# miha-stopar/Plonky3-mobile

Hardware: AMD Instinct MI355X
Metric: fib_air proofs/sec (higher is better)
Workload: dtype u32 (BabyBear Montgomery, 31-bit modular)

## Files before the change

### plonky3-mobile_amd/csrc/c_api.hip

```cpp
#include "../../include/p3hip.h"

#include <atomic>
#include <chrono>
#include <condition_variable>
#include <mutex>
#include <deque>
#include <thread>
#include <cctype>
#include <cstdio>
#include <cstring>

#include "bb31.hip.h"
#include "challenger.h"
#include "common.h"
#include "mmcs.h"
#include "prover.h"
#include "pcs_verifier_dev.h"
#include "verifier_dev.h"
#include "rng.h"

namespace p3 {
bool take_error(std::string* out);
}
using namespace p3;
// ... 257 lines not shown
        int rc = get_context(&cx);
        if (rc) return rc;
        return fib_trace((hipStream_t)stream, a, b, n, d_out);
    });
}

int p3hip_poseidon2_permute_dev(uint32_t* d_states, size_t n, void* stream) {
    return guarded([&]() -> int {
        if (n && !d_states) return fail(ERR_BAD_ARG, "null state pointer");
        if (misaligned(d_states, 4)) return fail(ERR_BAD_ARG, "poseidon2_permute: d_states must be 4-byte aligned");
        Context* cx;
        int rc = get_context(&cx);
        if (rc) return rc;
        if (misaligned(d_states, 16)) return poseidon2_permute_states_variant((hipStream_t)stream, d_states, n, 3);
        return poseidon2_permute_states((hipStream_t)stream, d_states, n);
    });
}
int p3hip_poseidon2_permute(uint32_t* states, size_t n) {
    return guarded([&]() -> int {
        if (!n) return OK;
        if (!states) return fail(ERR_BAD_ARG, "null state pointer");
        Context* cx;
        int rc = get_context(&cx);
        if (rc) return rc;
        hipStream_t stream = nullptr;
        rc = cx->ws(stream, 2).reserve(n * 64);
        if (rc) return rc;
        P3_HIP(hipMemcpy(cx->ws(stream, 2).ptr, states, n * 64, hipMemcpyHostToDevice));
        rc = poseidon2_permute_states(stream, cx->ws(stream, 2).as<uint32_t>(), n);
        if (rc) return rc;
        P3_HIP(hipMemcpy(states, cx->ws(stream, 2).ptr, n * 64, hipMemcpyDeviceToHost));
        return OK;
    });
}

int p3hip_poseidon2_permute_variant_dev(uint32_t* d_states, size_t n, int variant, void* stream) {
    return guarded([&]() -> int {
        if (n && !d_states) return fail(ERR_BAD_ARG, "null state pointer");
        if (variant < 0 || variant > 3)
            return fail(ERR_BAD_ARG, "poseidon2 variant: 0 = int32, 1 = fp64, 2 = fp64 one state per quad, 3 = int32 one state per 16 lanes");
        if (n > ((size_t)1 << 26)) return fail(ERR_BAD_ARG, "poseidon2 variant: at most 2^26 states per call");
        if (!n) return OK;
        if (misaligned(d_states, variant == 3 ? 4 : 16))
            return fail(ERR_BAD_ARG, "poseidon2 variant: d_states must be 16-byte aligned (4-byte for variant 3)");
        Context* cx;
        int rc = get_context(&cx);
        if (rc) return rc;
        return poseidon2_permute_states_variant((hipStream_t)stream, d_states, n, variant);
    });
}
int p3hip_poseidon2_f64_probe_dev(const double* d_in, uint32_t* d_out, size_t n, int mode, void* stream) {
    return guarded([&]() -> int {
        if (n && (!d_in || !d_out)) return fail(ERR_BAD_ARG, "null pointer");
        if (mode < 0 || mode > 3)
            return fail(ERR_BAD_ARG, "probe mode: 0 = permutation, 1 = internal rounds, 2 = reduce, 3 = permutation, one state per quad");
        if (n > ((size_t)1 << 26)) return fail(ERR_BAD_ARG, "probe: at most 2^26 states per call");
        if (!n) return OK;
        if (misaligned(d_in, 8)) return fail(ERR_BAD_ARG, "probe: d_in holds doubles and must be 8-byte aligned");
        Context* cx;
        int rc = get_context(&cx);
        if (rc) return rc;
        return poseidon2_f64_probe((hipStream_t)stream, d_in, d_out, n, mode);
    });
}
int p3hip_field_probe_dev(int op, const void* d_in, void* d_out, size_t n, void* stream) {
    return guarded([&]() -> int { return field_probe((hipStream_t)stream, op, d_in, d_out, n); });
}
int p3hip_field_probe_host(int op, const void* in, void* out, size_t n) {
    return guarded([&]() -> int { return field_probe_host(op, in, out, n); });
}

}
struct p3hip_tree {
    Tree* t;
};
extern "C" {

static int commit_async_kind(int kind, const uint32_t* const* d_mats, const size_t* heights, const size_t* widths,
                             size_t n_mats, p3hip_tree_t** tree_out, void* stream) {
    return guarded([&]() -> int {
        if (!tree_out) return fail(ERR_BAD_ARG, "mmcs_commit: null tree_out");
        Context* cx;
        int rc = get_context(&cx);
        if (rc) return rc;
        Tree* t = nullptr;
        rc = mmcs_commit((hipStream_t)stream, d_mats, heights, widths, n_mats, &t, nullptr, nullptr, kind, nullptr, cx->profile);
        if (rc) return rc;
        *tree_out = new p3hip_tree{t};
        return OK;
    });
}
int p3hip_mmcs_commit_async_dev(const uint32_t* const* d_mats, const size_t* heights, const size_t* widths,
                                size_t n_mats, p3hip_tree_t** tree_out, void* stream) {
    return commit_async_kind(HASH_POSEIDON2, d_mats, heights, widths, n_mats, tree_out, stream);
}
int p3hip_mmcs_commit_hash_dev(int hash, const uint32_t* const* d_mats, const size_t* heights, const size_t* widths,
                               size_t n_mats, uint32_t root_out[8], p3hip_tree_t** tree_out, void* stream) {
    if (!root_out) return fail(ERR_BAD_ARG, "mmcs_commit: null root_out");
    int rc = commit_async_kind(hash, d_mats, heights, widths, n_mats, tree_out, stream);
    if (rc) return rc;
    rc = p3hip_mmcs_root(*tree_out, root_out, stream);
    if (rc) { p3hip_mmcs_free(*tree_out); *tree_out = nullptr; }
    return rc;
}
size_t p3hip_mmcs_layer_words(size_t max_height) { return mmcs_layer_words(max_height); }
int p3hip_mmcs_commit_into_dev(int hash, const uint32_t* const* d_mats, const size_t* heights, const size_t* widths, size_t n_mats,
                               uint32_t* d_layers, p3hip_tree_t** tree_out, void* stream) {
    return guarded([&]() -> int {
// ... 1124 lines not shown
```

### plonky3-mobile_amd/csrc/mmcs.hip

```cpp
#include <algorithm>

#include "common.h"
#include "mmcs.h"
#include "poseidon2.hip.h"
#include "poseidon2_coop.hip.h"
#include "poseidon2_f64.hip.h"
#include "poseidon2_q4.hip.h"
#include "keccak.hip.h"

namespace p3 {

constexpr int MAX_CLASS_MATS = 16;

struct RowSet {
    const uint32_t* ptr[MAX_CLASS_MATS];
    uint32_t width[MAX_CLASS_MATS];
    uint32_t stride[MAX_CLASS_MATS];
    uint32_t count;
    uint32_t total;
};

__device__ __forceinline__ void load_digest(const uint32_t* p, uint32_t* out8) {
    const uint4* q = reinterpret_cast<const uint4*>(p);
    uint4 a = q[0], b = q[1];
// ... 40 lines not shown
    if (r >= n_rows) return;
    uint32_t s[16];
    sponge_row(rs, r, s);
    store_digest(digests + r * 8, s);
}

__global__ void __launch_bounds__(256) compress_layer_kernel(const uint32_t* prev, uint32_t* next, uint64_t n_out,
                                                             RowSet rs, uint32_t inject) {
    if (gridDim.x <= 512u) P3_LATENCY_BOUND_KERNEL();
    uint64_t i = (uint64_t)blockIdx.x * blockDim.x + threadIdx.x;
    if (i >= n_out) return;
    uint32_t s[16];
    load_digest(prev + i * 16, s);
    load_digest(prev + i * 16 + 8, s + 8);
    p2::permute(s);
    if (inject) {
        uint32_t h[16];
        sponge_row(rs, i, h);
#pragma unroll
        for (int k = 0; k < 8; k++) s[8 + k] = h[k];
        p2::permute(s);
    }
    store_digest(next + i * 8, s);
}

__global__ void __launch_bounds__(256) tree_top_kernel(uint32_t* layer0, uint32_t n0) {
    P3_LATENCY_BOUND_KERNEL();
    extern __shared__ __attribute__((aligned(16))) uint32_t lds[];
    const uint32_t tid = threadIdx.x;
    for (uint32_t i = tid; i < n0 * 8; i += blockDim.x) lds[i] = layer0[i];
    __syncthreads();
    uint32_t* out = layer0 + (size_t)n0 * 8;
    for (uint32_t n = n0; n > 1; n >>= 1) {
        uint32_t half = n >> 1;
        uint32_t s[16];
        bool act = tid < half;
        if (act) {
#pragma unroll
            for (int k = 0; k < 16; k++) s[k] = lds[tid * 16 + k];
            p2::permute(s);
        }
        __syncthreads();
        if (act) {
#pragma unroll
            for (int k = 0; k < 8; k++) lds[tid * 8 + k] = s[k];
            store_digest(out + tid * 8, s);
        }
        __syncthreads();
        out += (size_t)half * 8;
    }
}


__global__ void __launch_bounds__(256) leaf_hash_f64_kernel(const uint32_t* mat, uint32_t width, uint64_t n_rows, uint32_t* digests) {
    if (gridDim.x <= 512u) P3_LATENCY_BOUND_KERNEL();
    uint64_t r = (uint64_t)blockIdx.x * blockDim.x + threadIdx.x;
    if (r >= n_rows) return;
    double s[16];
#pragma unroll
    for (int i = 0; i < 16; i++) s[i] = 0.0;
    const uint32_t* row = mat + r * width;
    for (uint32_t k = 0; k < width; k += 8) {
#pragma unroll
        for (int i = 0; i < 8; i++)
            if (k + i < width) s[i] = p2f::load_elem(row[k + i]);
        p2f::permute(s);
        if (k + 8 < width) {
#pragma unroll
            for (int i = 0; i < 16; i++) s[i] = p2f::reduce(s[i]);
        }
    }
    uint32_t d[8];
    const p2f::MagicRegs smk = p2f::magic_regs();
#pragma unroll
    for (int i = 0; i < 8; i++) d[i] = p2f::store_elem(s[i], smk);
    store_digest(digests + r * 8, d);
}
__global__ void __launch_bounds__(256) compress_layer_q4_kernel(const uint32_t* prev, uint32_t* next, uint64_t n_out, uint32_t prio) {
    if (prio) P3_LATENCY_BOUND_KERNEL();
    const uint32_t q = threadIdx.x & 3u;
    const uint64_t i = ((uint64_t)blockIdx.x * blockDim.x + threadIdx.x) >> 2;
    const bool act = i < n_out;
    const p2q::LaneConsts lc = p2q::lane_consts(q);
    double s[4] = {0.0, 0.0, 0.0, 0.0};
    if (act) {
        const uint4 w = *reinterpret_cast<const uint4*>(prev + i * 16 + 4 * q);
        s[0] = p2f::load_elem(w.x); s[1] = p2f::load_elem(w.y); s[2] = p2f::load_elem(w.z); s[3] = p2f::load_elem(w.w);
    }
    p2q::permute(s, lc, q == 0);
    if (act && q < 2) {
        const p2f::MagicRegs smk = p2f::magic_regs();
        *reinterpret_cast<uint4*>(next + i * 8 + 4 * q) =
            make_uint4(p2f::store_elem(s[0], smk), p2f::store_elem(s[1], smk), p2f::store_elem(s[2], smk), p2f::store_elem(s[3], smk));
    }
}
__global__ void __launch_bounds__(256) leaf_hash_q4_kernel(const uint32_t* mat, uint32_t width, uint64_t n_rows, uint32_t* digests, uint32_t prio) {
    if (prio) P3_LATENCY_BOUND_KERNEL();
    const uint32_t q = threadIdx.x & 3u;
    const uint64_t r = ((uint64_t)blockIdx.x * blockDim.x + threadIdx.x) >> 2;
    const bool act = r < n_rows;
    const p2q::LaneConsts lc = p2q::lane_consts(q);
    double s[4] = {0.0, 0.0, 0.0, 0.0};
    const uint32_t* row = mat + (act ? r : 0) * width;
    for (uint32_t k = 0; k < width; k += 8) {
        if (act && q < 2) {
#pragma unroll
            for (uint32_t i = 0; i < 4; i++)
                if (k + 4 * q + i < width) s[i] = p2f::load_elem(row[k + 4 * q + i]);
        }
        p2q::permute(s, lc, q == 0);
        if (k + 8 < width) {
#pragma unroll
            for (int i = 0; i < 4; i++) s[i] = p2f::reduce(s[i]);
        }
    }
    if (act && q < 2) {
        const p2f::MagicRegs smk = p2f::magic_regs();
        *reinterpret_cast<uint4*>(digests + r * 8 + 4 * q) =
            make_uint4(p2f::store_elem(s[0], smk), p2f::store_elem(s[1], smk), p2f::store_elem(s[2], smk), p2f::store_elem(s[3], smk));
    }
}
constexpr uint32_t LEAF_WIDE_CHUNK = 32, LEAF_WIDE_STRIDE = 36;
__global__ void __launch_bounds__(256) leaf_hash_f64_wide_kernel(const uint32_t* mat, uint32_t width, uint64_t n_rows, uint32_t* digests) {
    __shared__ __attribute__((aligned(16))) uint32_t tile[256 * LEAF_WIDE_STRIDE];
    const uint32_t tid = threadIdx.x, col = tid & 31u, rsub = tid >> 5;
    const uint64_t r0 = (uint64_t)blockIdx.x * 256u, r = r0 + tid;
    double s[16];
#pragma unroll
    for (int i = 0; i < 16; i++) s[i] = 0.0;
// ... 145 lines not shown
    p2::permute(s);
#pragma unroll
    for (int k = 0; k < 4; k++) q[k] = make_uint4(s[4 * k], s[4 * k + 1], s[4 * k + 2], s[4 * k + 3]);
}


__global__ void __launch_bounds__(256, 8) poseidon2_permute_f64_kernel(uint32_t* states, uint64_t n) {
    uint64_t i = (uint64_t)blockIdx.x * blockDim.x + threadIdx.x;
    if (i >= n) return;
    double s[16];
    uint4* q = reinterpret_cast<uint4*>(states + i * 16);
#pragma unroll
    for (int k = 0; k < 4; k++) {
        uint4 v = q[k];
        s[4 * k] = p2f::load_elem(v.x); s[4 * k + 1] = p2f::load_elem(v.y); s[4 * k + 2] = p2f::load_elem(v.z); s[4 * k + 3] = p2f::load_elem(v.w);
    }
    p2f::permute(s);
#pragma unroll
    for (int k = 0; k < 4; k++)
        q[k] = make_uint4(p2f::store_elem(s[4 * k]), p2f::store_elem(s[4 * k + 1]), p2f::store_elem(s[4 * k + 2]), p2f::store_elem(s[4 * k + 3]));
}

__global__ void poseidon2_f64_probe_kernel(const double* in, uint32_t* out, uint64_t n, int mode) {
    uint64_t i = (uint64_t)blockIdx.x * blockDim.x + threadIdx.x;
    if (i >= n) return;
    double s[16];
#pragma unroll
    for (int k = 0; k < 16; k++) s[k] = in[i * 16 + k];
    if (mode == 0) p2f::permute(s);
    else if (mode == 1) p2f::internal_rounds(s, p2f::magic_regs());
    else {
#pragma unroll
        for (int k = 0; k < 16; k++) s[k] = p2f::reduce(s[k]);
    }
#pragma unroll
    for (int k = 0; k < 16; k++) out[i * 16 + k] = p2f::store_elem(s[k]);
}
__global__ void __launch_bounds__(256) poseidon2_q4_probe_kernel(const double* in, uint32_t* out, uint64_t n) {
    const uint32_t q = threadIdx.x & 3u;
    const uint64_t i = ((uint64_t)blockIdx.x * blockDim.x + threadIdx.x) >> 2;
    const bool act = i < n;
    const p2q::LaneConsts lc = p2q::lane_consts(q);
    double s[4] = {0.0, 0.0, 0.0, 0.0};
    if (act) {
#pragma unroll
        for (int k = 0; k < 4; k++) s[k] = in[i * 16 + 4 * q + k];
    }
    p2q::permute(s, lc, q == 0);
    if (act) {
#pragma unroll
        for (int k = 0; k < 4; k++) out[i * 16 + 4 * q + k] = p2f::store_elem(s[k]);
    }
}
int poseidon2_f64_probe(hipStream_t stream, const double* d_in, uint32_t* d_out, uint64_t n, int mode) {
    if (!n) return OK;
    if (mode == 3) hipLaunchKernelGGL(poseidon2_q4_probe_kernel, dim3((uint32_t)((n * 4 + 255) / 256)), dim3(256), 0, stream, d_in, d_out, n);
    else hipLaunchKernelGGL(poseidon2_f64_probe_kernel, dim3((uint32_t)((n + 255) / 256)), dim3(256), 0, stream, d_in, d_out, n, mode);
    P3_HIP(hipGetLastError());
    return OK;
}
__global__ void __launch_bounds__(256) poseidon2_permute_q4_kernel(uint32_t* states, uint64_t n) {
    const uint32_t q = threadIdx.x & 3u;
    const uint64_t i = ((uint64_t)blockIdx.x * blockDim.x + threadIdx.x) >> 2;
    const bool act = i < n;
    const p2q::LaneConsts lc = p2q::lane_consts(q);
    double s[4] = {0.0, 0.0, 0.0, 0.0};
    uint4* mine = reinterpret_cast<uint4*>(states + (act ? i : 0) * 16 + 4 * q);
    if (act) {
        const uint4 w = *mine;
        s[0] = p2f::load_elem(w.x); s[1] = p2f::load_elem(w.y); s[2] = p2f::load_elem(w.z); s[3] = p2f::load_elem(w.w);
    }
    p2q::permute(s, lc, q == 0);
    if (act) {
        const p2f::MagicRegs smk = p2f::magic_regs();
        *mine = make_uint4(p2f::store_elem(s[0], smk), p2f::store_elem(s[1], smk), p2f::store_elem(s[2], smk), p2f::store_elem(s[3], smk));
    }
}
__global__ void __launch_bounds__(256) poseidon2_permute_coop_kernel(uint32_t* states, uint64_t n) {
    const uint32_t lane16 = threadIdx.x & 15;
    const p2c::LaneConst lc = p2c::lane_constants(lane16);
    const uint64_t i = ((uint64_t)blockIdx.x * blockDim.x + threadIdx.x) >> 4;
    const bool act = i < n;
    uint32_t v = act ? states[i * 16 + lane16] : 0u;
    v = p2c::permute(v, lc);
    if (act) states[i * 16 + lane16] = v;
}
int poseidon2_permute_states_variant(hipStream_t stream, uint32_t* d_states, uint64_t n, int variant) {
    if (!n) return OK;
    if (variant == 3) hipLaunchKernelGGL(poseidon2_permute_coop_kernel, dim3((uint32_t)((n * 16 + 255) / 256)), dim3(256), 0, stream, d_states, n);
    else if (variant == 2) hipLaunchKernelGGL(poseidon2_permute_q4_kernel, dim3((uint32_t)((n * 4 + 255) / 256)), dim3(256), 0, stream, d_states, n);
    else if (variant == 1) hipLaunchKernelGGL(poseidon2_permute_f64_kernel, dim3((uint32_t)((n + 255) / 256)), dim3(256), 0, stream, d_states, n);
    else hipLaunchKernelGGL(poseidon2_permute_kernel, dim3((uint32_t)((n + 255) / 256)), dim3(256), 0, stream, d_states, n);
    P3_HIP(hipGetLastError());
    return OK;
}

int poseidon2_permute_states(hipStream_t stream, uint32_t* d_states, uint64_t n) {
    return poseidon2_permute_states_variant(stream, d_states, n, 1);
}

__device__ __forceinline__ uint32_t rowset_elem(const RowSet& rs, uint64_t r, uint32_t k, uint32_t& m, uint32_t& base) {
    while (k - base >= rs.width[m]) { base += rs.width[m]; m++; }
    return rs.ptr[m][r * rs.stride[m] + (k - base)];
}
__device__ __forceinline__ void keccak_sponge_row(const RowSet& rs, uint64_t r, uint64_t (&st)[25]) {
#pragma unroll
    for (int i = 0; i < 25; i++) st[i] = 0;
    const uint32_t n = rs.total, n64 = (n + 1) / 2;
    uint32_t m = 0, base = 0;
// ... 435 lines not shown
    const uint64_t KCOOP_IN = profile == PROFILE_LATENCY ? (1ull << 12) : (1ull << 10);
    constexpr uint32_t KCOOP_CHUNK_LOG = 4;
    constexpr uint64_t KLANE_CHUNK = 1ull << 7;
    if (kind == HASH_KECCAK) {
        RowSet rs0 = make_rowset(*t, maxh);
        if (rs0.count == 1 && rs0.width[0] >= 68 && rs0.stride[0] == rs0.width[0])
            hipLaunchKernelGGL(keccak_leaf_wide_kernel, dim3((uint32_t)((maxh + 255) / 256)), dim3(256), 0, stream, rs0.ptr[0], rs0.width[0], maxh,
                               t->layers);
        else if (!launch_keccak_leaf_salted(stream, rs0, maxh, t->layers))
            hipLaunchKernelGGL(keccak_leaf_kernel, dim3((uint32_t)((maxh + 255) / 256)), dim3(256), 0, stream, rs0, maxh, t->layers);
        P3_HIP(hipGetLastError());
        for (size_t l = 1; l < t->layer_len.size(); l++) {
            uint64_t len = t->layer_len[l];
            RowSet rs = make_rowset(*t, len);
            if (len < COOP_MAX && !rs.count) {
                const uint64_t n_in = t->layer_len[l - 1];
                const bool coop = n_in <= KCOOP_IN;
                uint32_t levels = 0;
                while (levels < (coop ? KCOOP_CHUNK_LOG : 11u) && l + levels < t->layer_len.size() && !has_height(*t, t->layer_len[l + levels])) levels++;
                if (!coop) while (levels > 1 && (n_in >> levels) < KCOOP_IN) levels--;
                const uint32_t chunk = (uint32_t)std::min<uint64_t>(n_in, coop ? 1ull << KCOOP_CHUNK_LOG : KLANE_CHUNK);
                while ((1u << levels) > chunk) levels--;
                if (coop)
                    hipLaunchKernelGGL(keccak_tree_levels_coop_kernel, dim3((uint32_t)(n_in / chunk)), dim3(std::max<uint32_t>(64, chunk * 32)), 0,
                                       stream, t->layers + t->layer_off[l - 1], (uint32_t)n_in, chunk, levels, root_copy);
                else
                    hipLaunchKernelGGL(keccak_tree_levels_kernel, dim3((uint32_t)(n_in / chunk)), dim3(std::max<uint32_t>(64, chunk / 2)),
                                       (size_t)chunk * 32, stream, t->layers + t->layer_off[l - 1], (uint32_t)n_in, chunk, levels, root_copy);
                P3_HIP(hipGetLastError());
                if (t->layer_len[l + levels - 1] == 1) t->root_copied = root_copy != nullptr;
                l += levels - 1;
                continue;
            }
            hipLaunchKernelGGL(keccak_compress_kernel, dim3((uint32_t)((len + 255) / 256)), dim3(256), 0, stream,
                               t->layers + t->layer_off[l - 1], t->layers + t->layer_off[l], len, rs, rs.count > 0 ? 1u : 0u);
            P3_HIP(hipGetLastError());
        }
        *out = t.release();
        return OK;
    }
    {
        RowSet rs = make_rowset(*t, maxh);
        const bool dense1 = rs.count == 1 && rs.stride[0] == rs.width[0];
        if (dense1 && maxh < COOP_MAX && maxh * 16 <= 0x7fffffffull) {
            hipLaunchKernelGGL(leaf_coop_kernel, dim3((uint32_t)((maxh * 16 + 255) / 256)), dim3(256), 0, stream, rs.ptr[0],
                               rs.width[0], (uint32_t)maxh, t->layers);
        } else if (dense1 && maxh <= Q4_MAX && rs.width[0] <= 64 && (reinterpret_cast<uintptr_t>(t->layers) & 15u) == 0) {
            hipLaunchKernelGGL(leaf_hash_q4_kernel, dim3((uint32_t)((maxh * 4 + 255) / 256)), dim3(256), 0, stream, rs.ptr[0], rs.width[0], maxh,
                               t->layers, Q4_PRIO);
        } else if (dense1 && rs.width[0] >= 64) {
            hipLaunchKernelGGL(leaf_hash_f64_wide_kernel, dim3((uint32_t)((maxh + 255) / 256)), dim3(256), 0, stream, rs.ptr[0],
                               rs.width[0], maxh, t->layers);
        } else if (dense1) {
            hipLaunchKernelGGL(leaf_hash_f64_kernel, dim3((uint32_t)((maxh + 255) / 256)), dim3(256), 0, stream, rs.ptr[0],
                               rs.width[0], maxh, t->layers);
        } else if ((maxh >= COOP_MAX || (rs.count == 1 && !dense1))) {
            hipLaunchKernelGGL(leaf_hash_f64_rowset_kernel, dim3((uint32_t)((maxh + 255) / 256)), dim3(256), 0, stream, rs, maxh, t->layers);
        } else {
            hipLaunchKernelGGL(leaf_hash_kernel, dim3((uint32_t)((maxh + 255) / 256)), dim3(256), 0, stream, rs, maxh, t->layers);
        }
        P3_HIP(hipGetLastError());
    }
    for (size_t l = 1; l < t->layer_len.size();) {
        uint64_t len = t->layer_len[l];
        RowSet rs = make_rowset(*t, len);
        bool inject = rs.count > 0;
        if (!inject && len < COOP_MAX) {
            uint32_t levels = 0;
            while (levels < COOP_CHUNK_LOG && l + levels < t->layer_len.size() && !has_height(*t, t->layer_len[l + levels])) levels++;
            uint64_t n_in = t->layer_len[l - 1];
            uint32_t chunk = (uint32_t)std::min<uint64_t>(n_in, 1ull << COOP_CHUNK_LOG);
            while ((1u << levels) > chunk) levels--;
            uint32_t blocks = (uint32_t)(n_in / chunk);
            uint32_t threads = std::max<uint32_t>(64, chunk * 8);
            bool makes_root = t->layer_len[l + levels - 1] == 1;
            hipLaunchKernelGGL(tree_levels_coop_kernel, dim3(blocks), dim3(threads), 0, stream, t->layers + t->layer_off[l - 1],
                               (uint32_t)n_in, chunk, levels, makes_root ? root_copy : nullptr);
            P3_HIP(hipGetLastError());
            if (makes_root) t->root_copied = root_copy != nullptr;
            l += levels;
            continue;
        }
        if (!inject && len <= Q4_MAX) {
            hipLaunchKernelGGL(compress_layer_q4_kernel, dim3((uint32_t)((len * 4 + 255) / 256)), dim3(256), 0, stream,
                               t->layers + t->layer_off[l - 1], t->layers + t->layer_off[l], len, Q4_PRIO);
        } else if (!inject) {
            hipLaunchKernelGGL(compress_layer_f64_kernel, dim3((uint32_t)((len + 255) / 256)), dim3(256), 0, stream,
                               t->layers + t->layer_off[l - 1], t->layers + t->layer_off[l], len);
        } else {
            hipLaunchKernelGGL(compress_layer_kernel, dim3((uint32_t)((len + 255) / 256)), dim3(256), 0, stream,
                               t->layers + t->layer_off[l - 1], t->layers + t->layer_off[l], len, rs, inject ? 1u : 0u);
        }
        P3_HIP(hipGetLastError());
        l++;
    }
    *out = t.release();
    return OK;
}

int mmcs_root(hipStream_t stream, const Tree& t, uint32_t root_out[8]) {
    P3_HIP(hipMemcpyAsync(root_out, t.layers + t.layer_off.back(), 32, hipMemcpyDeviceToHost, stream));
    P3_HIP(hipStreamSynchronize(stream));
    return OK;
}

static OpenArgs make_open_args(const Tree& t) {
    OpenArgs a{};
    a.n_mats = (uint32_t)t.mats.size();
// ... 47 lines not shown
```

### plonky3-mobile_amd/csrc/poseidon2_f64.hip.h

```cpp
#pragma once
#include "poseidon2.hip.h"

namespace p2f {

constexpr double PD = 2013265921.0;
constexpr double PINV = 1.0 / 2013265921.0;

__device__ __forceinline__ double mulmod(double a, double b) {
    double h = a * b;
    double l = __fma_rn(a, b, -h);
    double q = __builtin_rint(h * PINV);
    double r = __fma_rn(-q, PD, h);
    return r + l;
}
constexpr double PM1 = 2013265920.0;
__device__ __forceinline__ double mulmod_p(double a, double b, double aP) {
    double q = __builtin_rint(b * aP);
    double t = __fma_rn(a, b, -(q * PM1));
    return t - q;
}
__device__ __forceinline__ double reduce(double x) {
    return __fma_rn(-__builtin_rint(x * PINV), PD, x);
}
__device__ __forceinline__ double add_scaled_pow2(double tot, double x, double inv) {
// ... 88 lines not shown
    auto internal_round = [&](int r) {
        s[0] = sbox7(s[0] + d_c.in[r], mk, npm1, pinv);
        const double ti = (((s[0] + s[1]) + (s[2] + s[4])) + ((s[5] + s[7]) + (s[8] + s[12]))) + s[15];
        const double tf = ((s[3] + s[6]) + (s[9] + s[10])) + ((s[11] + s[13]) + s[14]);
        const double tot = reduce(ti + fold_dyadic(tf));
        s[0] = __fma_rn(s[0], -2.0, tot);
        s[1] = tot + s[1];
        s[2] = __fma_rn(s[2], 2.0, tot);
        s[3] = __fma_rn(s[3], 0.5, tot);
        s[4] = __fma_rn(s[4], k3, tot);
        s[5] = __fma_rn(s[5], 4.0, tot);
        s[6] = __fma_rn(s[6], -0.5, tot);
        s[7] = __fma_rn(s[7], -k3, tot);
        s[8] = __fma_rn(s[8], -4.0, tot);
        s[9] = __fma_rn(s[9], i256, tot);
        s[10] = __fma_rn(s[10], i4, tot);
        s[11] = __fma_rn(s[11], i8, tot);
        s[12] = __fma_rn(s[12], -k15, tot);
        s[13] = __fma_rn(s[13], -i256, tot);
        s[14] = __fma_rn(s[14], -i16, tot);
        s[15] = __fma_rn(s[15], k15, tot);
        if (FOLD_K1 >> r & 1) { s[3] = fold_dyadic(s[3]); s[6] = fold_dyadic(s[6]); }
        if (FOLD_K8 >> r & 1) { s[9] = fold_dyadic(s[9]); s[13] = fold_dyadic(s[13]); }
        if (FOLD_K2 >> r & 1) s[10] = fold_dyadic(s[10]);
        if (FOLD_K3 >> r & 1) s[11] = fold_dyadic(s[11]);
        if (FOLD_K4 >> r & 1) s[14] = fold_dyadic(s[14]);
        if (FOLD_X2 >> r & 1) { s[1] = reduce(s[1]); s[2] = reduce(s[2]); }
        if (FOLD_X4 >> r & 1) { s[4] = reduce(s[4]); s[5] = reduce(s[5]); s[7] = reduce(s[7]); s[8] = reduce(s[8]); }
        if (FOLD_X15 >> r & 1) { s[12] = reduce(s[12]); s[15] = reduce(s[15]); }
    };
#pragma unroll
    for (int r = 0; r < 13; r++) internal_round(r);
}

__device__ __forceinline__ void permute(double (&s)[16]) {
    const MagicRegs mk = magic_regs();
    const double npm1 = d_c.neg_pm1, pinv = d_c.pinv;
    external_linear(s);
    _Pragma("clang loop unroll(disable)")
    for (int r = 0; r < 4; r++) {
#pragma unroll
        for (int i = 0; i < 16; i++) s[i] = sbox7(s[i] + d_c.ext[r][i], mk, npm1, pinv);
        external_linear(s);
    }
    internal_rounds(s, mk);
    _Pragma("clang loop unroll(disable)")
    for (int r = 4; r < 8; r++) {
#pragma unroll
        for (int i = 0; i < 16; i++) s[i] = sbox7(s[i] + d_c.ext[r][i], mk, npm1, pinv);
        external_linear(s);
    }
}

__device__ __forceinline__ double load_elem(uint32_t monty) { return (double)bb::from_monty(monty); }
constexpr double R_MOD_P = 268435454.0;
constexpr double R_MOD_P_OVER_P = 268435454.0 / 2013265921.0;
__device__ __forceinline__ uint32_t store_elem(double v, const MagicRegs& k) {
    const double r = mulmod_m(R_MOD_P, v, R_MOD_P_OVER_P, k, d_c.neg_pm1);
    const uint32_t w = (uint32_t)(int32_t)r;
    return min(w, w + bb::P);
}
__device__ __forceinline__ uint32_t store_elem(double v) { return store_elem(v, magic_regs()); }

}
```

### plonky3-mobile_amd/csrc/prover.hip

```cpp
#include <chrono>
#include <cstddef>
#include <deque>
#include <memory>
#include <cstring>

#include "bb31.hip.h"
#include "challenger.h"
#include "common.h"
#include "keccak.hip.h"
#include "mmcs.h"
#include "poseidon2.hip.h"
#include "poseidon2_f64.hip.h"
#include "prover.h"
#include "rng.h"
#include "rng_dev.hip.h"
#include "transcript.hip.h"

namespace p3 {

using bb::Ext;

__device__ __forceinline__ uint32_t tl(const TwoLevelTable& t, uint32_t e) {
    return bb::mul(t.lo[e & ((1u << t.T) - 1u)], t.hi[e >> t.T]);
}
// ... 170 lines not shown
    uint32_t* ro;
    const DevState* ds;
    uint32_t big;
};
__global__ void __launch_bounds__(256) reduced_openings_kernel(ReducedArgs a) {
    uint32_t j = blockIdx.x * blockDim.x + threadIdx.x;
    if (j >= a.big) return;
    const DevState* __restrict__ ds = a.ds;
    uint2 t = a.lde_t[j];
    uint4 q = a.lde_q[j];
    Ext u, w;
#pragma unroll
    for (int c = 0; c < 4; c++) {
        u.c[c] = bb::add(bb::add(bb::dot2(ds->alp[4].c[c], q.x, ds->alp[5].c[c], q.y), bb::dot2(ds->alp[6].c[c], q.z, ds->alp[7].c[c], q.w)),
                         bb::mul(ds->alp[1].c[c], t.y));
        w.c[c] = bb::dot2(ds->alp[2].c[c], t.x, ds->alp[3].c[c], t.y);
    }
    u.c[0] = bb::add(u.c[0], t.x);
    Ext e0 = ld_ext(a.d0 + 4 * (size_t)j), e1 = ld_ext(a.d1 + 4 * (size_t)j);
    Ext r = bb::add(bb::mul(bb::sub(ds->y02, u), e0), bb::mul(bb::sub(ds->y1, w), e1));
    st_ext(a.ro + 4 * (size_t)j, r);
}

__global__ void __launch_bounds__(256) fri_fold_kernel(TwoLevelTable inv_roots , const uint32_t* in,
                                                       uint32_t* out, uint32_t half, uint32_t log_half,
                                                       const DevState* __restrict__ ds, uint32_t round, uint32_t one_half) {
    if (gridDim.x <= 512u) P3_LATENCY_BOUND_KERNEL();
    uint32_t i = blockIdx.x * blockDim.x + threadIdx.x;
    if (i >= half) return;
    const Ext half_beta = ds->half_beta[round];
    Ext lo = ld_ext(in + 8 * (size_t)i), hi = ld_ext(in + 8 * (size_t)i + 4);
    uint32_t p = tl(inv_roots, brev(i, log_half));
    Ext s = bb::scale(bb::add(lo, hi), one_half);
    Ext d = bb::mul(bb::scale(half_beta, p), bb::sub(lo, hi));
    st_ext(out + 4 * (size_t)i, bb::add(s, d));
}

__global__ void __launch_bounds__(256) fri_fold_rollin_kernel(TwoLevelTable inv_roots , const uint32_t* in,
                                                              const uint32_t* __restrict__ ro, uint32_t* out, uint32_t half,
                                                              uint32_t log_half, const DevState* __restrict__ ds, uint32_t round,
                                                              uint32_t one_half) {
    if (gridDim.x <= 512u) P3_LATENCY_BOUND_KERNEL();
    uint32_t i = blockIdx.x * blockDim.x + threadIdx.x;
    if (i >= half) return;
    const Ext half_beta = ds->half_beta[round];
    const Ext beta2 = bb::sqr(bb::add(half_beta, half_beta));
    Ext lo = ld_ext(in + 8 * (size_t)i), hi = ld_ext(in + 8 * (size_t)i + 4), e = ld_ext(ro + 4 * (size_t)i);
    uint32_t p = tl(inv_roots, brev(i, log_half));
    Ext s = bb::scale(bb::add(lo, hi), one_half);
    Ext d = bb::mul(bb::scale(half_beta, p), bb::sub(lo, hi));
    st_ext(out + 4 * (size_t)i, bb::add(bb::add(s, d), bb::mul(beta2, e)));
}

__global__ void __launch_bounds__(256, 8) grind_kernel(DevState* ds, uint32_t mask, uint32_t base) {
    uint32_t w = base + blockIdx.x * blockDim.x + threadIdx.x;
    if (w >= bb::P) return;
    if (base + blockIdx.x * blockDim.x > *(volatile uint32_t*)&ds->grind_result) return;
    const uint32_t pos = ds->n_in;
    double s[16];
#pragma unroll
    for (int i = 0; i < 16; i++) s[i] = p2f::load_elem((i < 8 && (uint32_t)i < pos) ? ds->inb[i & 7] : ds->st[i]);
#pragma unroll
    for (int i = 0; i < 8; i++) s[i] = (i == (int)pos) ? (double)w : s[i];
    p2f::permute(s);
    if ((bb::from_monty(p2f::store_elem(s[7])) & mask) == 0) atomicMin(&ds->grind_result, w);
}

__global__ void __launch_bounds__(256) grind_keccak_kernel(DevState* ds, uint32_t mask, uint32_t base) {
    uint32_t w = base + blockIdx.x * blockDim.x + threadIdx.x;
    if (w >= bb::P) return;
    if (base + blockIdx.x * blockDim.x > *(volatile uint32_t*)&ds->grind_result) return;
    const KeccakGrindArgs& a = ds->kgrind;
    const uint32_t wm = bb::to_monty(w);
    uint64_t st[25];
#pragma unroll
    for (int i = 0; i < 25; i++) st[i] = a.state[i];
    for (uint32_t blk = 0; blk < a.n_blocks; blk++) {
#pragma unroll
        for (int i = 0; i < 17; i++) {
            uint64_t lane = a.block[blk][i];
            const int32_t rel = (int32_t)(a.wpos) - (int32_t)(blk * 136 + i * 8);
            if (rel > -4 && rel < 8) {
                const uint64_t v = (uint64_t)wm;
                lane ^= rel >= 0 ? (v << (8 * rel)) : (v >> (8 * -rel));
            }
            st[i] ^= lane;
        }
        if (blk + 1 == a.n_blocks) kk::permute_digest(st);
        else kk::permute(st);
    }
    bool ok = false;
#pragma unroll
    for (int t = 0; t < 8; t++) {
        const uint64_t lane = st[3 - t / 2];
        const uint32_t hi_or_lo = (t & 1) ? (uint32_t)lane : (uint32_t)(lane >> 32);
        const uint32_t v = __builtin_bswap32(hi_or_lo) & 0x7fffffffu;
        if (v < bb::P) { ok = (v & mask) == 0; break; }
    }
    if (ok) atomicMin(&ds->grind_result, w);
}

constexpr uint32_t QTREE_MAX_MATS = 8;
struct QTree {
    const uint32_t* mat[QTREE_MAX_MATS];
    uint32_t width[QTREE_MAX_MATS];
    uint32_t stride[QTREE_MAX_MATS];
    uint32_t n_mats;
    const uint32_t* layers;
    uint32_t log_height, shift, slot_off;
    uint32_t mshift[QTREE_MAX_MATS];
};
__global__ void query_gather_kernel(const QTree* trees, const uint32_t* indices, uint32_t slot_words, uint32_t* out) {
    P3_LATENCY_BOUND_KERNEL();
    const QTree& t = trees[blockIdx.y];
    const uint64_t index = (indices[blockIdx.x] >> t.shift) & ((1ull << t.log_height) - 1ull);
    uint32_t* dst = out + (size_t)blockIdx.x * slot_words + t.slot_off;
    uint32_t off = 0;
    for (uint32_t m = 0; m < t.n_mats; m++) {
        const uint64_t row = index >> t.mshift[m];
        for (uint32_t c = threadIdx.x; c < t.width[m]; c += blockDim.x) dst[off + c] = t.mat[m][row * t.stride[m] + c];
        off += t.width[m];
    }
    uint64_t base = 0, len = 1ull << t.log_height;
    for (uint32_t i = 0; i < t.log_height; i++) {
        const uint64_t sib = (index >> i) ^ 1;
        if (threadIdx.x < 8) dst[off + i * 8 + threadIdx.x] = t.layers[base + sib * 8 + threadIdx.x];
        base += len * 8;
        len >>= 1;
    }
}

struct StageLayout {
    uint32_t root_t = 0, root_q = 8, opened = 16, froots = 48, fpoly = 0, witness = 0, status = 0, qidx = 0, slots = 0, words = 0;
};
struct TsArgs {
    DevState* ds;
    uint32_t* ps;
    int kind;
    StageLayout lay;
};
struct TsPis {
    uint32_t w[3];
    uint32_t given;
};

__global__ void __launch_bounds__(64) ts_begin_kernel(TsArgs a, const uint32_t* trace, uint32_t n, uint32_t log_n, TsPis given) {
    P3_LATENCY_BOUND_KERNEL();
    __shared__ KState ks;
    DevChal ch;
    ch.begin(a.kind, a.ds, &ks, true);
    uint32_t pis[3];
    if (given.given) {
// ... 355 lines not shown
               uint32_t root_slot, size_t mat_stride = 0, hipStream_t on = nullptr) {
        hipStream_t cs = on ? on : stream;
        const uint32_t* mp[QTREE_MAX_MATS]; size_t hh[QTREE_MAX_MATS], ww[QTREE_MAX_MATS], ss[QTREE_MAX_MATS];
        size_t k = 0;
        for (size_t i = 0; i < n; i++, k++) {
            mp[k] = mats[i]; hh[k] = height; ww[k] = widths[i]; ss[k] = mat_stride ? mat_stride : widths[i];
            if (salt_words) { k++; mp[k] = salts[i]; hh[k] = height; ww[k] = ss[k] = salt_words; }
        }
        Tree* tp = nullptr;
        int r = mmcs_commit(cs, mp, hh, ww, k, &tp, layers, pstage + root_slot, hash, ss, profile);
        if (r) return r;
        std::unique_ptr<Tree> t(tp);
        if (!t->root_copied) P3_HIP(hipMemcpyAsync(pstage + root_slot, t->layers + t->layer_off.back(), 32, hipMemcpyDeviceToDevice, cs));
        return OK;
    }
    int fri_rounds(Context& cx, const TsArgs& ts, uint32_t r_end, const uint32_t* const* rollin = nullptr) {
        const uint32_t one_half = bb::inv(bb::to_monty(2));
        const size_t row = 8;
        int rc;
        for (uint32_t r = 0; r < r_end; r++) {
            const uint32_t log_half = log_big - 1 - r, half = 1u << log_half;
            uint32_t* vec = fri_vec + fri_vec_off[r];
            uint32_t* salts = salt_words ? fri_salts + fri_salt_off[r] : nullptr;
            if ((rc = commit(1, &vec, &row, &salts, half, fri_layers + fri_layer_off[r], lay.froots + 8 * r))) return rc;
            hipLaunchKernelGGL(ts_fri_round_kernel, dim3(1), dim3(64), 0, stream, ts, r, one_half);
            P3_HIP(hipGetLastError());
            TwoLevelTable inv_roots;
            if ((rc = cx.get_root_table(stream, log_half + 1, true, &inv_roots))) return rc;
            if (rollin && rollin[r])
                hipLaunchKernelGGL(fri_fold_rollin_kernel, dim3((half + 255) / 256), dim3(256), 0, stream, inv_roots, vec, rollin[r],
                                   fri_vec + fri_vec_off[r + 1], half, log_half, ts.ds, r, one_half);
            else
                hipLaunchKernelGGL(fri_fold_kernel, dim3((half + 255) / 256), dim3(256), 0, stream, inv_roots, vec, fri_vec + fri_vec_off[r + 1],
                                   half, log_half, ts.ds, r, one_half);
            P3_HIP(hipGetLastError());
        }
        return OK;
    }
    int fri_final(Context& cx, const TsArgs& ts) {
        const uint32_t fpl = 1u << fp.log_final_poly_len;
        int rc;
        if ((rc = bit_reverse_rows(stream, fri_vec + fri_vec_off[n_rounds], fp_ev, fpl, 4))) return rc;
        if ((rc = ntt_dft(cx, stream, fp_ev, pstage + lay.fpoly, fpl, 4, true))) return rc;
        hipLaunchKernelGGL(ts_final_kernel, dim3(1), dim3(64), 0, stream, ts, fpl, pow_mask());
        P3_HIP(hipGetLastError());
        return OK;
    }

    uint32_t pow_mask() const { return (1u << fp.proof_of_work_bits) - 1u; }
    uint32_t grind_range(uint32_t first_log) const {
        return 1u << std::min<uint32_t>(std::max<uint32_t>(first_log ? first_log : fp.proof_of_work_bits + 4, 8), 24);
    }
    int grind(const TsArgs& ts, uint64_t base, uint32_t count) {
        if (hash == HASH_KECCAK) hipLaunchKernelGGL(grind_keccak_kernel, dim3(count / 256), dim3(256), 0, stream, ts.ds, pow_mask(), (uint32_t)base);
        else hipLaunchKernelGGL(grind_kernel, dim3(count / 256), dim3(256), 0, stream, ts.ds, pow_mask(), (uint32_t)base);
        P3_HIP(hipGetLastError());
        return OK;
    }
    int grind_start(const TsArgs& ts) {
        const uint32_t first_log = grind_first_log(), batch = grind_range(first_log);
        const uint32_t head = first_log ? batch : std::min<uint32_t>(batch, 1u << std::max<uint32_t>(fp.proof_of_work_bits + 1, 8));
        int rc;
        if ((rc = grind(ts, 0, head))) return rc;
        if (batch > head && (rc = grind(ts, head, batch - head))) return rc;
        return OK;
    }
    int queries(const TsArgs& ts, uint32_t* host, size_t words) {
        const uint32_t nq = fp.num_queries;
        hipLaunchKernelGGL(ts_queries_kernel, dim3(1), dim3(64), 0, stream, ts, nq, log_big, fp.proof_of_work_bits, qidx);
        P3_HIP(hipGetLastError());
        if (nq) {
            hipLaunchKernelGGL(query_gather_kernel, dim3(nq, (uint32_t)trees.size()), dim3(64), 0, stream, qtrees, qidx, (uint32_t)slot_words,
                               pstage + lay.slots);
            P3_HIP(hipGetLastError());
        }
        P3_HIP(hipMemcpyAsync(host, pstage, words * 4, hipMemcpyDeviceToHost, stream));
        return OK;
    }
    int continue_grind(const TsArgs& ts, uint32_t* host, size_t words) {
        uint32_t batch = grind_range(grind_first_log()), found = 0xffffffffu;
        int rc;
        for (uint64_t base = batch; base < bb::P && found == 0xffffffffu; base += batch) {
            batch = std::min<uint32_t>(batch * 4, 1u << 24);
            if ((rc = grind(ts, base, batch))) return rc;
            P3_HIP(hipMemcpyAsync(&found, &ts.ds->grind_result, 4, hipMemcpyDeviceToHost, stream));
            P3_HIP(hipStreamSynchronize(stream));
        }
        if (found == 0xffffffffu) return fail(ERR_INTERNAL, "grind: no proof-of-work witness found");
        if ((rc = queries(ts, host, words))) return rc;
        P3_HIP(hipStreamSynchronize(stream));
        return OK;
    }

    void put_fri(std::vector<uint8_t>& pf, const uint32_t* hp) const {
        const StageLayout& L = lay;
        const uint32_t nq = fp.num_queries, fpl = 1u << fp.log_final_poly_len, n_inputs = (uint32_t)trees.size() - n_rounds;
        put_u32(pf, n_rounds); put_words(pf, hp + L.froots, (size_t)n_rounds * 8);
        put_u32(pf, nq);
        for (uint32_t q = 0; q < nq; q++) {
            const uint32_t* slot = hp + L.slots + (size_t)q * slot_words;
            put_u32(pf, n_inputs);
            for (uint32_t i = 0; i < n_inputs; i++) {
                const QTree& t = trees[i];
                put_opening(pf, slot, salt_words ? t.n_mats / 2 : t.n_mats, t.width, salt_words, t.log_height);
            }
            put_u32(pf, n_rounds);
            for (uint32_t r = 0; r < n_rounds; r++) {
                const uint32_t lh = log_big - 1 - r, idx = hp[L.qidx + q] >> r;
                put_words(pf, slot + 4 * ((idx ^ 1) & 1), 4);
                if (salt_words) { put_u32(pf, salt_words); put_words(pf, slot + 8, salt_words); }
                put_u32(pf, lh); put_words(pf, slot + 8 + salt_words, (size_t)lh * 8);
                slot += 8 + salt_words + (size_t)lh * 8;
            }
        }
        put_u32(pf, fpl);
        put_words(pf, hp + L.fpoly, (size_t)fpl * 4);
        put_u32(pf, hp[L.witness]);
    }
};
// ... 304 lines not shown
```

Measured before the change: 564.8.

## Specialize Poseidon2 leaf hashing for narrow widths and use persistent grind kernels

Adds a permute_open variant that skips the final external linear layer and computes only the first 8 output lanes, plus mat4 specializations that exploit known-zero trailing lanes. Leaf hashing is templated on width 1..8, so sparse inputs avoid wasted arithmetic. Grinding now uses a persistent grid capped at 128 workgroups, with a grid-stride loop and a relaxed atomic early-exit check, and the two-stage head/tail grind launch becomes a single launch. New probe modes expose the open-form permutation for testing. The risks are lower grind parallelism and correctness errors in the hand-derived sparse matrix formulas.

```diff
diff --git a/plonky3-mobile_amd/csrc/c_api.hip b/plonky3-mobile_amd/csrc/c_api.hip
--- a/plonky3-mobile_amd/csrc/c_api.hip
+++ b/plonky3-mobile_amd/csrc/c_api.hip
@@ -333,8 +333,10 @@
 int p3hip_poseidon2_f64_probe_dev(const double* d_in, uint32_t* d_out, size_t n, int mode, void* stream) {
     return guarded([&]() -> int {
         if (n && (!d_in || !d_out)) return fail(ERR_BAD_ARG, "null pointer");
-        if (mode < 0 || mode > 3)
-            return fail(ERR_BAD_ARG, "probe mode: 0 = permutation, 1 = internal rounds, 2 = reduce, 3 = permutation, one state per quad");
+        const bool open_form = (mode >= 33 && mode <= 40) || mode == 48;
+        if ((mode < 0 || mode > 3) && !open_form)
+            return fail(ERR_BAD_ARG, "probe mode: 0 = permutation, 1 = internal rounds, 2 = reduce, 3 = permutation, one state per quad, "
+                                     "32 + NZ (NZ in 1..8 or 16) = permutation of a state with NZ leading non-zero lanes, words 0..7 out");
         if (n > ((size_t)1 << 26)) return fail(ERR_BAD_ARG, "probe: at most 2^26 states per call");
         if (!n) return OK;
         if (misaligned(d_in, 8)) return fail(ERR_BAD_ARG, "probe: d_in holds doubles and must be 8-byte aligned");
diff --git a/plonky3-mobile_amd/csrc/mmcs.hip b/plonky3-mobile_amd/csrc/mmcs.hip
--- a/plonky3-mobile_amd/csrc/mmcs.hip
+++ b/plonky3-mobile_amd/csrc/mmcs.hip
@@ -116,29 +116,58 @@
 }
 
 
-__global__ void __launch_bounds__(256) leaf_hash_f64_kernel(const uint32_t* mat, uint32_t width, uint64_t n_rows, uint32_t* digests) {
+template <uint32_t W>
+__global__ void __launch_bounds__(256, 8) leaf_hash_f64_kernel(const uint32_t* mat, uint32_t width, uint64_t n_rows, uint32_t* digests) {
     if (gridDim.x <= 512u) P3_LATENCY_BOUND_KERNEL();
     uint64_t r = (uint64_t)blockIdx.x * blockDim.x + threadIdx.x;
     if (r >= n_rows) return;
+    const p2f::MagicRegs mk = p2f::magic_regs();
     double s[16];
 #pragma unroll
     for (int i = 0; i < 16; i++) s[i] = 0.0;
-    const uint32_t* row = mat + r * width;
-    for (uint32_t k = 0; k < width; k += 8) {
+    if constexpr (W != 0) {
+        const uint32_t* row = mat + r * W;
+#pragma unroll
+        for (int i = 0; i < (int)W; i++) s[i] = p2f::load_elem(row[i]);
+        p2f::permute_open<(int)W>(s, mk);
+    } else if (width != 0) {
+        const uint32_t* row = mat + r * width;
+        uint32_t k = 0;
+        for (; k + 8 < width; k += 8) {
+#pragma unroll
+            for (int i = 0; i < 8; i++) s[i] = p2f::load_elem(row[k + i]);
+            p2f::permute_open(s, mk);
+            p2f::external_linear(s);
+#pragma unroll
+            for (int i = 0; i < 16; i++) s[i] = p2f::reduce(s[i]);
+        }
 #pragma unroll
         for (int i = 0; i < 8; i++)
             if (k + i < width) s[i] = p2f::load_elem(row[k + i]);
-        p2f::permute(s);
-        if (k + 8 < width) {
-#pragma unroll
-            for (int i = 0; i < 16; i++) s[i] = p2f::reduce(s[i]);
-        }
-    }
+        p2f::permute_open(s, mk);
+    }
+    p2f::external_linear_lo8(s);
     uint32_t d[8];
-    const p2f::MagicRegs smk = p2f::magic_regs();
-#pragma unroll
-    for (int i = 0; i < 8; i++) d[i] = p2f::store_elem(s[i], smk);
+#pragma unroll
+    for (int i = 0; i < 8; i++) d[i] = p2f::store_elem(s[i], mk);
     store_digest(digests + r * 8, d);
+}
+template <uint32_t W>
+static void launch_leaf_hash_f64_w(hipStream_t stream, const uint32_t* mat, uint32_t width, uint64_t n_rows, uint32_t* digests) {
+    hipLaunchKernelGGL(leaf_hash_f64_kernel<W>, dim3((uint32_t)((n_rows + 255) / 256)), dim3(256), 0, stream, mat, width, n_rows, digests);
+}
+static void launch_leaf_hash_f64(hipStream_t stream, const uint32_t* mat, uint32_t width, uint64_t n_rows, uint32_t* digests) {
+    switch (width) {
+        case 1: return launch_leaf_hash_f64_w<1>(stream, mat, width, n_rows, digests);
+        case 2: return launch_leaf_hash_f64_w<2>(stream, mat, width, n_rows, digests);
+        case 3: return launch_leaf_hash_f64_w<3>(stream, mat, width, n_rows, digests);
+        case 4: return launch_leaf_hash_f64_w<4>(stream, mat, width, n_rows, digests);
+        case 5: return launch_leaf_hash_f64_w<5>(stream, mat, width, n_rows, digests);
+        case 6: return launch_leaf_hash_f64_w<6>(stream, mat, width, n_rows, digests);
+        case 7: return launch_leaf_hash_f64_w<7>(stream, mat, width, n_rows, digests);
+        case 8: return launch_leaf_hash_f64_w<8>(stream, mat, width, n_rows, digests);
+        default: return launch_leaf_hash_f64_w<0>(stream, mat, width, n_rows, digests);
+    }
 }
 __global__ void __launch_bounds__(256) compress_layer_q4_kernel(const uint32_t* prev, uint32_t* next, uint64_t n_out, uint32_t prio) {
     if (prio) P3_LATENCY_BOUND_KERNEL();
@@ -390,9 +419,39 @@
         for (int k = 0; k < 4; k++) out[i * 16 + 4 * q + k] = p2f::store_elem(s[k]);
     }
 }
+template <int NZ>
+__global__ void __launch_bounds__(256, 8) poseidon2_f64_open_probe_kernel(const double* in, uint32_t* out, uint64_t n) {
+    uint64_t i = (uint64_t)blockIdx.x * blockDim.x + threadIdx.x;
+    if (i >= n) return;
+    const p2f::MagicRegs mk = p2f::magic_regs();
+    double s[16];
+#pragma unroll
+    for (int k = 0; k < 16; k++) s[k] = k < NZ ? in[i * 16 + k] : 0.0;
+    p2f::permute_open<NZ>(s, mk);
+    p2f::external_linear_lo8(s);
+#pragma unroll
+    for (int k = 0; k < 16; k++) out[i * 16 + k] = k < 8 ? p2f::store_elem(s[k], mk) : 0u;
+}
+template <int NZ>
+static void launch_open_probe(hipStream_t stream, const double* d_in, uint32_t* d_out, uint64_t n) {
+    hipLaunchKernelGGL(poseidon2_f64_open_probe_kernel<NZ>, dim3((uint32_t)((n + 255) / 256)), dim3(256), 0, stream, d_in, d_out, n);
+}
 int poseidon2_f64_probe(hipStream_t stream, const double* d_in, uint32_t* d_out, uint64_t n, int mode) {
     if (!n) return OK;
-    if (mode == 3) hipLaunchKernelGGL(poseidon2_q4_probe_kernel, dim3((uint32_t)((n * 4 + 255) / 256)), dim3(256), 0, stream, d_in, d_out, n);
+    if (mode >= 32) {
+        switch (mode - 32) {
+            case 1: launch_open_probe<1>(stream, d_in, d_out, n); break;
+            case 2: launch_open_probe<2>(stream, d_in, d_out, n); break;
+            case 3: launch_open_probe<3>(stream, d_in, d_out, n); break;
+            case 4: launch_open_probe<4>(stream, d_in, d_out, n); break;
+            case 5: launch_open_probe<5>(stream, d_in, d_out, n); break;
+            case 6: launch_open_probe<6>(stream, d_in, d_out, n); break;
+            case 7: launch_open_probe<7>(stream, d_in, d_out, n); break;
+            case 8: launch_open_probe<8>(stream, d_in, d_out, n); break;
+            case 16: launch_open_probe<16>(stream, d_in, d_out, n); break;
+            default: return fail(ERR_BAD_ARG, "probe mode");
+        }
+    } else if (mode == 3) hipLaunchKernelGGL(poseidon2_q4_probe_kernel, dim3((uint32_t)((n * 4 + 255) / 256)), dim3(256), 0, stream, d_in, d_out, n);
     else hipLaunchKernelGGL(poseidon2_f64_probe_kernel, dim3((uint32_t)((n + 255) / 256)), dim3(256), 0, stream, d_in, d_out, n, mode);
     P3_HIP(hipGetLastError());
     return OK;
@@ -934,8 +993,7 @@
             hipLaunchKernelGGL(leaf_hash_f64_wide_kernel, dim3((uint32_t)((maxh + 255) / 256)), dim3(256), 0, stream, rs.ptr[0],
                                rs.width[0], maxh, t->layers);
         } else if (dense1) {
-            hipLaunchKernelGGL(leaf_hash_f64_kernel, dim3((uint32_t)((maxh + 255) / 256)), dim3(256), 0, stream, rs.ptr[0],
-                               rs.width[0], maxh, t->layers);
+            launch_leaf_hash_f64(stream, rs.ptr[0], rs.width[0], maxh, t->layers);
         } else if ((maxh >= COOP_MAX || (rs.count == 1 && !dense1))) {
             hipLaunchKernelGGL(leaf_hash_f64_rowset_kernel, dim3((uint32_t)((maxh + 255) / 256)), dim3(256), 0, stream, rs, maxh, t->layers);
         } else {
diff --git a/plonky3-mobile_amd/csrc/poseidon2_f64.hip.h b/plonky3-mobile_amd/csrc/poseidon2_f64.hip.h
--- a/plonky3-mobile_amd/csrc/poseidon2_f64.hip.h
+++ b/plonky3-mobile_amd/csrc/poseidon2_f64.hip.h
@@ -164,6 +164,74 @@
     }
 }
 
+template <int N>
+__device__ __forceinline__ void mat4_lead(double& a, double& b, double& c, double& d) {
+    static_assert(N >= 1 && N <= 4, "mat4_lead");
+    if constexpr (N == 4) {
+        mat4(a, b, c, d);
+    } else if constexpr (N == 3) {
+        const double t01 = a + b, t012 = t01 + c, t0112 = t012 + b;
+        const double nd = __fma_rn(a, 2.0, t012), nb = __fma_rn(c, 2.0, t0112);
+        const double na = t0112 + t01, nc = t012 + c;
+        a = na; b = nb; c = nc; d = nd;
+    } else if constexpr (N == 2) {
+        const double t01 = a + b, t011 = t01 + b;
+        const double nd = __fma_rn(a, 2.0, t01), na = t011 + t01;
+        a = na; b = t011; c = t01; d = nd;
+    } else {
+        const double a2 = a + a, a3 = a2 + a;
+        b = a; c = a; d = a3; a = a2;
+    }
+}
+template <int NZ>
+__device__ __forceinline__ void external_linear_lead(double (&s)[16]) {
+    static_assert(NZ >= 1 && NZ <= 8, "external_linear_lead");
+    if constexpr (NZ <= 4) {
+        mat4_lead<NZ>(s[0], s[1], s[2], s[3]);
+#pragma unroll
+        for (int k = 0; k < 4; k++) { s[4 + k] = s[k]; s[8 + k] = s[k]; s[12 + k] = s[k]; s[k] += s[k]; }
+    } else {
+        mat4(s[0], s[1], s[2], s[3]);
+        mat4_lead<NZ - 4>(s[4], s[5], s[6], s[7]);
+#pragma unroll
+        for (int k = 0; k < 4; k++) {
+            const double t = s[k] + s[4 + k];
+            s[8 + k] = t; s[12 + k] = t; s[k] += t; s[4 + k] += t;
+        }
+    }
+}
+__device__ __forceinline__ void external_linear_lo8(double (&s)[16]) {
+    double t[4];
+#pragma unroll
+    for (int k = 0; k < 4; k++) t[k] = (s[k] + s[k + 4]) + (s[k + 8] + s[k + 12]);
+    mat4(t[0], t[1], t[2], t[3]);
+    mat4(s[0], s[1], s[2], s[3]);
+    mat4(s[4], s[5], s[6], s[7]);
+#pragma unroll
+    for (int i = 0; i < 8; i++) s[i] += t[i & 3];
+}
+template <int NZ = 16>
+__device__ __forceinline__ void permute_open(double (&s)[16], const MagicRegs& mk) {
+    const double npm1 = d_c.neg_pm1, pinv = d_c.pinv;
+    if constexpr (NZ == 16) external_linear(s);
+    else external_linear_lead<NZ>(s);
+    _Pragma("clang loop unroll(disable)")
+    for (int r = 0; r < 4; r++) {
+#pragma unroll
+        for (int i = 0; i < 16; i++) s[i] = sbox7(s[i] + d_c.ext[r][i], mk, npm1, pinv);
+        external_linear(s);
+    }
+    internal_rounds(s, mk);
+    _Pragma("clang loop unroll(disable)")
+    for (int r = 4; r < 7; r++) {
+#pragma unroll
+        for (int i = 0; i < 16; i++) s[i] = sbox7(s[i] + d_c.ext[r][i], mk, npm1, pinv);
+        external_linear(s);
+    }
+#pragma unroll
+    for (int i = 0; i < 16; i++) s[i] = sbox7(s[i] + d_c.ext[7][i], mk, npm1, pinv);
+}
+
 __device__ __forceinline__ double load_elem(uint32_t monty) { return (double)bb::from_monty(monty); }
 constexpr double R_MOD_P = 268435454.0;
 constexpr double R_MOD_P_OVER_P = 268435454.0 / 2013265921.0;
diff --git a/plonky3-mobile_amd/csrc/prover.hip b/plonky3-mobile_amd/csrc/prover.hip
--- a/plonky3-mobile_amd/csrc/prover.hip
+++ b/plonky3-mobile_amd/csrc/prover.hip
@@ -246,24 +246,32 @@
     st_ext(out + 4 * (size_t)i, bb::add(bb::add(s, d), bb::mul(beta2, e)));
 }
 
-__global__ void __launch_bounds__(256, 8) grind_kernel(DevState* ds, uint32_t mask, uint32_t base) {
-    uint32_t w = base + blockIdx.x * blockDim.x + threadIdx.x;
-    if (w >= bb::P) return;
-    if (base + blockIdx.x * blockDim.x > *(volatile uint32_t*)&ds->grind_result) return;
-    const uint32_t pos = ds->n_in;
-    double s[16];
-#pragma unroll
-    for (int i = 0; i < 16; i++) s[i] = p2f::load_elem((i < 8 && (uint32_t)i < pos) ? ds->inb[i & 7] : ds->st[i]);
-#pragma unroll
-    for (int i = 0; i < 8; i++) s[i] = (i == (int)pos) ? (double)w : s[i];
-    p2f::permute(s);
-    if ((bb::from_monty(p2f::store_elem(s[7])) & mask) == 0) atomicMin(&ds->grind_result, w);
-}
-
-__global__ void __launch_bounds__(256) grind_keccak_kernel(DevState* ds, uint32_t mask, uint32_t base) {
-    uint32_t w = base + blockIdx.x * blockDim.x + threadIdx.x;
-    if (w >= bb::P) return;
-    if (base + blockIdx.x * blockDim.x > *(volatile uint32_t*)&ds->grind_result) return;
+constexpr uint32_t GRIND_WGS = 128;
+__device__ __forceinline__ bool grind_block_live(const DevState* ds, uint32_t blk_base) {
+    const uint32_t best = __hip_atomic_load(&ds->grind_result, __ATOMIC_RELAXED, __HIP_MEMORY_SCOPE_AGENT);
+    return blk_base <= (uint32_t)__builtin_amdgcn_readfirstlane((int)best);
+}
+__global__ void __launch_bounds__(256, 8) grind_kernel(DevState* ds, uint32_t mask, uint32_t base, uint32_t count) {
+    const uint32_t n_blocks = count / 256;
+    uint32_t w = base + blockIdx.x * 256 + threadIdx.x;
+    const p2f::MagicRegs mk = p2f::magic_regs();
+    for (uint32_t b = blockIdx.x; b < n_blocks; b += gridDim.x, w += gridDim.x * 256) {
+        if (!grind_block_live(ds, base + b * 256)) return;
+        if (w >= bb::P) continue;
+        asm volatile("" ::: "memory");
+        const uint32_t pos = ds->n_in;
+        double s[16];
+#pragma unroll
+        for (int i = 0; i < 16; i++) s[i] = p2f::load_elem((i < 8 && (uint32_t)i < pos) ? ds->inb[i & 7] : ds->st[i]);
+#pragma unroll
+        for (int i = 0; i < 8; i++) s[i] = (i == (int)pos) ? (double)w : s[i];
+        p2f::permute_open(s, mk);
+        p2f::external_linear_lo8(s);
+        if ((bb::from_monty(p2f::store_elem(s[7], mk)) & mask) == 0) atomicMin(&ds->grind_result, w);
+    }
+}
+
+__device__ __forceinline__ void grind_keccak_candidate(DevState* ds, uint32_t mask, uint32_t w) {
     const KeccakGrindArgs& a = ds->kgrind;
     const uint32_t wm = bb::to_monty(w);
     uint64_t st[25];
@@ -292,6 +300,16 @@
         if (v < bb::P) { ok = (v & mask) == 0; break; }
     }
     if (ok) atomicMin(&ds->grind_result, w);
+}
+__global__ void __launch_bounds__(256) grind_keccak_kernel(DevState* ds, uint32_t mask, uint32_t base, uint32_t count) {
+    const uint32_t n_blocks = count / 256;
+    for (uint32_t b = blockIdx.x; b < n_blocks; b += gridDim.x) {
+        const uint32_t blk_base = base + b * 256;
+        if (!grind_block_live(ds, blk_base)) return;
+        const uint32_t w = blk_base + threadIdx.x;
+        if (w >= bb::P) return;
+        grind_keccak_candidate(ds, mask, w);
+    }
 }
 
 constexpr uint32_t QTREE_MAX_MATS = 8;
@@ -753,19 +771,13 @@
         return 1u << std::min<uint32_t>(std::max<uint32_t>(first_log ? first_log : fp.proof_of_work_bits + 4, 8), 24);
     }
     int grind(const TsArgs& ts, uint64_t base, uint32_t count) {
-        if (hash == HASH_KECCAK) hipLaunchKernelGGL(grind_keccak_kernel, dim3(count / 256), dim3(256), 0, stream, ts.ds, pow_mask(), (uint32_t)base);
-        else hipLaunchKernelGGL(grind_kernel, dim3(count / 256), dim3(256), 0, stream, ts.ds, pow_mask(), (uint32_t)base);
+        const dim3 grid(std::min<uint32_t>(count / 256, GRIND_WGS));
+        if (hash == HASH_KECCAK) hipLaunchKernelGGL(grind_keccak_kernel, grid, dim3(256), 0, stream, ts.ds, pow_mask(), (uint32_t)base, count);
+        else hipLaunchKernelGGL(grind_kernel, grid, dim3(256), 0, stream, ts.ds, pow_mask(), (uint32_t)base, count);
         P3_HIP(hipGetLastError());
         return OK;
     }
-    int grind_start(const TsArgs& ts) {
-        const uint32_t first_log = grind_first_log(), batch = grind_range(first_log);
-        const uint32_t head = first_log ? batch : std::min<uint32_t>(batch, 1u << std::max<uint32_t>(fp.proof_of_work_bits + 1, 8));
-        int rc;
-        if ((rc = grind(ts, 0, head))) return rc;
-        if (batch > head && (rc = grind(ts, head, batch - head))) return rc;
-        return OK;
-    }
+    int grind_start(const TsArgs& ts) { return grind(ts, 0, grind_range(grind_first_log())); }
     int queries(const TsArgs& ts, uint32_t* host, size_t words) {
         const uint32_t nq = fp.num_queries;
         hipLaunchKernelGGL(ts_queries_kernel, dim3(1), dim3(64), 0, stream, ts, nq, log_big, fp.proof_of_work_bits, qidx);
```

New measurement: 548.7. -2.9%, worse.
